# d-justen/duckdb-polr

Measured on AMD Instinct MI355X. Metric: probe-tuples/s, higher is better.
Workload: dtype u64

## Files before the change

duckdb-polr_amd/csrc/polr_flat_device.h:

```cpp
#pragma once

#include <hip/hip_runtime.h>
#include <stdint.h>

#include <type_traits>

#include "polr_device.h"

#define FLAT_STEP0 512
#define FLAT_UNIT_MAX 65536u

template <int K>
__device__ __host__ constexpr int flat_sweep_f() {
	return K <= 2 ? 8 : 4;
}
template <int K>
__device__ __host__ constexpr int flat_qcap() {
	return 64 * flat_sweep_f<K>() - 1 + 512;
}
template <int K>
__device__ __host__ constexpr int flat_qoff(int pos) {
	return (pos - 1) * (flat_qcap<K>() + 1);
}
template <int K>
__device__ __host__ constexpr int flat_per_wave_dwords() {
	return K <= 1 ? 0 : ((K - 1) * (flat_qcap<K>() + 1) * 2 + 3) / 4;
}

struct FlatStage {
	const POLR_GLOBAL uint32_t *keys;
	const POLR_GLOBAL uint8_t *valid;
	const POLR_GLOBAL uint32_t *table;
	uint32_t kind_lds;
	uint32_t a, b;
	uint32_t out_slot;
};

__device__ __forceinline__ FlatStage flat_load_stage(const StageDesc *d_generic, uint32_t join_index) {
	const POLR_GLOBAL StageDesc *d = as_global(d_generic);
	FlatStage s;
	s.out_slot = 1u + join_index;
	s.keys = as_global(uniptr((const uint32_t *)d->key_data[0]));
	s.valid = as_global(uniptr(d->key_valid[0]));
	s.table = as_global(uniptr((const uint32_t *)d->table));
	const uint32_t kind = uni(d->kind);
	s.kind_lds = kind | (uni(d->lds_off1) << 8);
	s.a = kind == KIND_PERFECT ? uni((uint32_t)d->min_value) : uni((uint32_t)d->mask);
	s.b = uni((uint32_t)d->range);
	return s;
}

template <int K>
struct FlatCtx {
	uint32_t k, lane;
	FlatStage st[K];
	const POLR_GLOBAL uint32_t *sel;
	const POLR_LDS uint32_t *lds_tables;
	POLR_LDS uint16_t *q;
	uint32_t qsize[K], cnt[K];
	uint64_t unit_begin, in_pos, in_end;
	DevOut out;
	OutState os;
	POLR_LDS unsigned long long *fused_lds;
	uint4 pf0, pf1;
	uint64_t pf_pos;
};

template <int F>
__device__ __forceinline__ void flat_perfect_issue(const FlatStage &s, const POLR_LDS uint32_t *lds_tables, const uint32_t (&key)[F],
                                                   const bool (&act)[F], uint32_t (&idx)[F], uint32_t (&w)[F]) {
	const uint32_t lds_off1 = s.kind_lds >> 8;
	bool in[F];
#pragma unroll
	for (int i = 0; i < F; i++) {
		idx[i] = key[i] - s.a;
		in[i] = act[i] && idx[i] <= s.b;
		w[i] = 0;
	}
	if (lds_off1) {
		const POLR_LDS uint32_t *bits = lds_tables + (lds_off1 - 1u);
#pragma unroll
		for (int i = 0; i < F; i++) {
			if (in[i]) {
				w[i] = bits[idx[i] >> 5];
			}
		}
	} else {
#pragma unroll
		for (int i = 0; i < F; i++) {
			if (in[i]) {
				w[i] = s.table[idx[i] >> 5];
			}
		}
	}
}

template <int F>
__device__ __forceinline__ void flat_hash_lookup(const FlatStage &s, const uint32_t (&key)[F], const bool (&act)[F],
                                                 bool (&hit)[F]) {
	const POLR_GLOBAL uint32_t *tab = s.table;
#pragma unroll
	for (int h0 = 0; h0 < F; h0 += 4) {
		uint32_t group[4], first[4];
		bool searching[4];
		bool any = false;
		const uint32_t gmask = s.a >> 2;
#pragma unroll
		for (int i = 0; i < 4; i++) {
			const uint64_t h = polr_murmurhash64((uint64_t)key[h0 + i]) & (uint64_t)s.a;
			group[i] = (uint32_t)(h >> 2);
			first[i] = (uint32_t)(h & 3u);
			searching[i] = act[h0 + i];
			hit[h0 + i] = false;
			any = any || searching[i];
		}
		while (__ballot(any) != 0ull) {
			uint4 a[4], b[4];
#pragma unroll
			for (int i = 0; i < 4; i++) {
				if (searching[i]) {
					a[i] = load_global_x4(tab + (uint64_t)group[i] * 8);
					b[i] = load_global_x4(tab + (uint64_t)group[i] * 8 + 4);
				}
			}
			any = false;
#pragma unroll
			for (int i = 0; i < 4; i++) {
				if (searching[i]) {
					const uint32_t kk[4] = {a[i].x, a[i].z, b[i].x, b[i].z};
					const uint32_t rr[4] = {a[i].y, a[i].w, b[i].y, b[i].w};
#pragma unroll
					for (int j = 0; j < 4; j++) {
						if (searching[i] && (uint32_t)j >= first[i]) {
							if (rr[j] == S8_EMPTY_ROW) {
								searching[i] = false;
							} else if (kk[j] == key[h0 + i]) {
								hit[h0 + i] = true;
								searching[i] = false;
							}
						}
					}
					first[i] = 0;
					group[i] = (group[i] + 1) & gmask;
				}
				any = any || searching[i];
			}
		}
	}
}

template <int F>
__device__ __forceinline__ void flat_lookup(const FlatStage &s, const POLR_LDS uint32_t *lds_tables, const uint32_t (&key)[F],
                                            const bool (&act)[F], bool (&hit)[F]) {
	if ((s.kind_lds & 0xFFu) == KIND_PERFECT) {
		uint32_t idx[F], w[F];
		flat_perfect_issue<F>(s, lds_tables, key, act, idx, w);
#pragma unroll
		for (int i = 0; i < F; i++) {
			hit[i] = (w[i] >> (idx[i] & 31u)) & 1u;
		}
	} else {
		flat_hash_lookup<F>(s, key, act, hit);
	}
}

#ifndef POLR_FLAT_EMIT
#define POLR_FLAT_EMIT 0
#endif
template <int K>
__device__ __forceinline__ void flat_fused_accumulate(FlatCtx<K> &c, uint32_t row) {
	const FusedSink *f = c.out.fused;
	auto slot_row = [&](uint32_t slot) {
		uint32_t r = row;
#pragma unroll
		for (int p = 0; p < K; p++) {
			if (p < (int)c.k && c.st[p].out_slot == slot) {
				r = c.st[p].keys[row] - c.st[p].a;
			}
		}
		return r;
	};
	uint64_t g = 0;
	bool ok = true;
	for (uint32_t q = 0; q < f->groups.n; q++) {
		const DevGroupKey gk = f->groups.k[q];
		const uint32_t r = slot_row(gk.slot);
		if (gk.src.valid && !as_global(gk.src.valid)[r]) {
			ok = false;
			break;
		}
		const unsigned long long off = (unsigned long long)(load_col_cell(gk.src, r) - gk.min_value);
		if (off >= gk.n_values) {
			ok = false;
			break;
		}
		g = g * gk.n_values + off;
	}
	if (!ok) {
		__hip_atomic_fetch_add(f->dropped, 1ull, __ATOMIC_RELAXED, __HIP_MEMORY_SCOPE_AGENT);
		return;
	}
	const uint32_t n_aggs = f->aggs.n;
	const size_t at = g * (1u + 2u * n_aggs);
	unsigned long long *gcell = f->cells + (size_t)(blockIdx.x % f->n_tables) * f->words_per_table + at;
	POLR_LDS unsigned long long *lcell = c.fused_lds + at;
	const bool in_lds = c.fused_lds != nullptr;
	auto add = [&](uint32_t w, unsigned long long v) {
		if (in_lds) {
			__hip_atomic_fetch_add(&lcell[w], v, __ATOMIC_RELAXED, __HIP_MEMORY_SCOPE_WORKGROUP);
		} else {
			__hip_atomic_fetch_add(&gcell[w], v, __ATOMIC_RELAXED, __HIP_MEMORY_SCOPE_AGENT);
		}
	};
	add(0, 1ull);
	for (uint32_t a = 0; a < n_aggs; a++) {
		const DevAgg ag = f->aggs.a[a];
		if (ag.fn == POLR_DEV_AGG_COUNT_STAR) {
			continue;
		}
		const uint32_t r = slot_row(ag.slot);
		if (ag.src.valid) {
			if (!as_global(ag.src.valid)[r]) {
				continue;
			}
			add(2u + 2u * a, 1ull);
		}
		if (ag.fn == POLR_DEV_AGG_SUM) {
			add(1u + 2u * a, (unsigned long long)load_col_cell(ag.src, r));
		}
	}
}

template <int K>
__device__ __forceinline__ void flat_out_write(FlatCtx<K> &c, uint32_t pos, bool valid) {
	const uint64_t m = __ballot(valid);
	const uint32_t n = (uint32_t)__popcll(m);
	if (n == 0) {
		return;
	}
	POLR_GLOBAL uint32_t *ids = as_global(c.out.ids);
	uint32_t row = 0, id[K];
	if (valid) {
		const uint64_t tp = c.unit_begin + pos;
		row = c.sel ? c.sel[tp] : (uint32_t)tp;
	}
	if (c.out.fused) {
		if (valid) {
			flat_fused_accumulate<K>(c, row);
		}
		return;
	}
	if (valid) {
#pragma unroll
		for (int p = 0; p < K; p++) {
			id[p] = p < (int)c.k ? c.st[p].keys[row] - c.st[p].a : 0u;
		}
	}
	out_claim(c.out, c.os, c.lane, m, valid, [&](uint64_t place) {
		ids[place] = row;
#pragma unroll
		for (int p = 0; p < K; p++) {
			if (p < (int)c.k) {
				ids[(uint64_t)c.st[p].out_slot * c.out.slot_stride + place] = id[p];
			}
		}
	});
}

template <int K, int POS, int F>
__device__ __forceinline__ void flat_emit(FlatCtx<K> &c, const uint32_t (&pos)[F], const bool (&hit)[F]) {
	const bool last = POS + 1 >= K || POS + 1 == (int)c.k;
	uint32_t total = 0;
#if POLR_FLAT_EMIT
	if (last && c.os.emit) {
#pragma unroll 1
		for (int i = 0; i < F; i++) {
			uint32_t p_i = pos[0];
			bool h_i = hit[0];
#pragma unroll
			for (int j = 1; j < F; j++) {
				p_i = j == i ? pos[j] : p_i;
				h_i = j == i ? hit[j] : h_i;
			}
			flat_out_write<K>(c, p_i, h_i);
		}
	}
#endif
	if constexpr (POS + 1 < K) {
		POLR_LDS uint16_t *qq = c.q + flat_qoff<K>(POS + 1);
		uint32_t qs = c.qsize[POS + 1];
#pragma unroll
		for (int i = 0; i < F; i++) {
			const uint64_t m = __ballot(hit[i]);
			const uint32_t n = (uint32_t)__popcll(m);
			if (!last && hit[i]) {
				qq[qs + lane_rank(m)] = (uint16_t)pos[i];
			}
			qs += n;
			total += n;
		}
		if (!last) {
			c.qsize[POS + 1] = qs;
		}
	} else {
#pragma unroll
		for (int i = 0; i < F; i++) {
			total += (uint32_t)__popcll(__ballot(hit[i]));
		}
	}
	c.cnt[POS] += total;
}

template <int K>
__device__ __forceinline__ void flat_stage0(FlatCtx<K> &c) {
	constexpr int F = 4;
	const FlatStage &s = c.st[0];
	const uint64_t left = c.in_end - c.in_pos;
	const uint32_t n = left < FLAT_STEP0 ? (uint32_t)left : (uint32_t)FLAT_STEP0;
	const uint32_t upos = (uint32_t)(c.in_pos - c.unit_begin);
	const bool streamable = c.sel == nullptr && s.valid == nullptr && (c.in_pos & 3ull) == 0 && (((uint64_t)s.keys) & 15ull) == 0;
	if (n == FLAT_STEP0 && streamable) {
		const uint32_t base = (uint32_t)c.in_pos + 4u * c.lane;
		uint4 kk[2];
		if (c.pf_pos == c.in_pos) {
			kk[0] = c.pf0;
			kk[1] = c.pf1;
		} else {
			kk[0] = load_global_x4(s.keys + base);
			kk[1] = load_global_x4(s.keys + base + 256u);
		}
		if (c.in_end - c.in_pos >= 2ull * FLAT_STEP0) {
			c.pf0 = load_global_x4(s.keys + base + FLAT_STEP0);
			c.pf1 = load_global_x4(s.keys + base + FLAT_STEP0 + 256u);
			c.pf_pos = c.in_pos + FLAT_STEP0;
		} else {
			c.pf_pos = ~0ull;
		}
		c.in_pos += n;
#pragma unroll
		for (int h = 0; h < 2; h++) {
			const uint32_t key[F] = {kk[h].x, kk[h].y, kk[h].z, kk[h].w};
			uint32_t pos[F];
			bool act[F], hit[F];
#pragma unroll
			for (int i = 0; i < F; i++) {
				pos[i] = upos + 4u * c.lane + h * 256u + i;
				act[i] = true;
			}
			flat_lookup<F>(s, c.lds_tables, key, act, hit);
			flat_emit<K, 0, F>(c, pos, hit);
		}
		return;
	}
	c.pf_pos = ~0ull;
	const uint64_t pos0 = c.in_pos;
	c.in_pos += n;
#pragma unroll 1
	for (uint32_t h = 0; h * 256u < n; h++) {
		uint32_t pos[F], row[F], key[F];
		bool act[F], hit[F];
#pragma unroll
		for (int i = 0; i < F; i++) {
			const uint32_t off = h * 256u + c.lane + 64u * i;
			act[i] = off < n;
			pos[i] = upos + off;
			const uint64_t tp = pos0 + off;
			row[i] = act[i] ? (c.sel ? c.sel[tp] : (uint32_t)tp) : 0u;
		}
#pragma unroll
		for (int i = 0; i < F; i++) {
			key[i] = act[i] ? s.keys[row[i]] : 0u;
		}
		if (s.valid) {
#pragma unroll
			for (int i = 0; i < F; i++) {
				act[i] = act[i] && s.valid[row[i]] != 0;
			}
		}
		flat_lookup<F>(s, c.lds_tables, key, act, hit);
		flat_emit<K, 0, F>(c, pos, hit);
	}
}

template <int I, int N, class Fn>
__device__ __forceinline__ void flat_static_for(Fn &&fn) {
	if constexpr (I < N) {
		fn(std::integral_constant<int, I> {});
		flat_static_for<I + 1, N>(fn);
	}
}
template <int I, int N, class Fn>
__device__ __forceinline__ void flat_static_for_down(Fn &&fn) {
	if constexpr (I >= 1) {
		fn(std::integral_constant<int, I> {});
		flat_static_for_down<I - 1, N>(fn);
	}
}

template <int K>
__device__ __forceinline__ void flat_sweep(FlatCtx<K> &c) {
	constexpr int F = flat_sweep_f<K>();
	if constexpr (K > 1) {
		uint32_t pos[K - 1][F], key[K - 1][F], w[K - 1][F];
		flat_static_for<1, K>([&](auto P) {
			constexpr int p = decltype(P)::value;
			if (p < (int)c.k) {
				const FlatStage &s = c.st[p];
				const uint32_t qs = c.qsize[p];
				const uint32_t n = qs < (uint32_t)(64 * F) ? qs : (uint32_t)(64 * F);
				const uint32_t base = qs - n;
				const POLR_LDS uint16_t *qq = c.q + flat_qoff<K>(p);
				uint32_t row[F];
#pragma unroll
				for (int i = 0; i < F; i++) {
					const uint32_t off = c.lane + 64u * i;
					pos[p - 1][i] = off < n ? (uint32_t)qq[base + off] : 0xFFFFFFFFu;
				}
				c.qsize[p] = base;
				if (c.sel) {
#pragma unroll
					for (int i = 0; i < F; i++) {
						row[i] = pos[p - 1][i] != 0xFFFFFFFFu ? c.sel[c.unit_begin + pos[p - 1][i]] : 0u;
					}
				} else {
#pragma unroll
					for (int i = 0; i < F; i++) {
						row[i] = (uint32_t)c.unit_begin + pos[p - 1][i];
					}
				}
#pragma unroll
				for (int i = 0; i < F; i++) {
					key[p - 1][i] = pos[p - 1][i] != 0xFFFFFFFFu ? s.keys[row[i]] : 0u;
				}
				if (s.valid) {
#pragma unroll
					for (int i = 0; i < F; i++) {
						if (pos[p - 1][i] != 0xFFFFFFFFu && s.valid[row[i]] == 0) {
							pos[p - 1][i] = 0xFFFFFFFFu;
						}
					}
				}
			}
		});
		flat_static_for<1, K>([&](auto P) {
			constexpr int p = decltype(P)::value;
			if (p < (int)c.k && (c.st[p].kind_lds & 0xFFu) == KIND_PERFECT) {
				const FlatStage &s = c.st[p];
				const uint32_t lds_off1 = s.kind_lds >> 8;
				bool in[F];
#pragma unroll
				for (int i = 0; i < F; i++) {
					const uint32_t idx = key[p - 1][i] - s.a;
					in[i] = pos[p - 1][i] != 0xFFFFFFFFu && idx <= s.b;
					key[p - 1][i] = idx;
					w[p - 1][i] = 0;
				}
				if (lds_off1) {
					const POLR_LDS uint32_t *bits = c.lds_tables + (lds_off1 - 1u);
#pragma unroll
					for (int i = 0; i < F; i++) {
						if (in[i]) {
							w[p - 1][i] = bits[key[p - 1][i] >> 5];
						}
					}
				} else {
#pragma unroll
					for (int i = 0; i < F; i++) {
						if (in[i]) {
							w[p - 1][i] = s.table[key[p - 1][i] >> 5];
						}
					}
				}
#pragma unroll
				for (int i = 0; i < F; i++) {
					key[p - 1][i] &= 31u;
				}
			}
		});
		flat_static_for<1, K>([&](auto P) {
			constexpr int p = decltype(P)::value;
			if (p < (int)c.k && (c.st[p].kind_lds & 0xFFu) != KIND_PERFECT) {
				bool act[F], hit[F];
#pragma unroll
				for (int i = 0; i < F; i++) {
					act[i] = pos[p - 1][i] != 0xFFFFFFFFu;
				}
				flat_hash_lookup<F>(c.st[p], key[p - 1], act, hit);
#pragma unroll
				for (int i = 0; i < F; i++) {
					w[p - 1][i] = hit[i] ? 1u : 0u;
					key[p - 1][i] = 0;
				}
			}
		});
		flat_static_for_down<K - 1, K>([&](auto P) {
			constexpr int p = decltype(P)::value;
			if (p < (int)c.k) {
				bool hit[F];
#pragma unroll
				for (int i = 0; i < F; i++) {
					hit[i] = (w[p - 1][i] >> key[p - 1][i]) & 1u;
				}
				flat_emit<K, p, F>(c, pos[p - 1], hit);
			}
		});
	}
}

template <int K>
__device__ __forceinline__ void flat_run_source(FlatCtx<K> &c) {
	while (true) {
		bool deep_full = false;
#pragma unroll
		for (int p = 1; p < K; p++) {
			if (p < (int)c.k) {
				deep_full = deep_full || c.qsize[p] >= (uint32_t)(64 * flat_sweep_f<K>());
			}
		}
		if (deep_full) {
			flat_sweep<K>(c);
		} else if (c.in_pos < c.in_end) {
			flat_stage0<K>(c);
		} else {
			return;
		}
	}
}

template <int K>
__device__ __forceinline__ void flat_run_drain(FlatCtx<K> &c) {
	while (true) {
		bool deep_any = false;
#pragma unroll
		for (int p = 1; p < K; p++) {
			if (p < (int)c.k) {
				deep_any = deep_any || c.qsize[p] > 0;
			}
		}
		if (!deep_any) {
			return;
		}
		flat_sweep<K>(c);
	}
}

template <int K>
__device__ __forceinline__ void flat_prefetch_unit(FlatCtx<K> &c, uint64_t begin, uint32_t count) {
	const FlatStage &s = c.st[0];
	const bool streamable = c.sel == nullptr && s.valid == nullptr && (begin & 3ull) == 0 && (((uint64_t)s.keys) & 15ull) == 0;
	if (count >= (uint32_t)FLAT_STEP0 && streamable) {
		const uint32_t base = (uint32_t)begin + 4u * c.lane;
		c.pf0 = load_global_x4(s.keys + base);
		c.pf1 = load_global_x4(s.keys + base + 256u);
		c.pf_pos = begin;
	}
}
```

duckdb-polr_amd/csrc/polr_pool.hip:

```cpp
#include <hip/hip_runtime.h>
#include <stdint.h>
#include <stddef.h>

#include "polr_device.h"
#include "polr_mpx_device.h"

#ifndef POLR_K
#error "compile with -DPOLR_K=<compiled stage count>"
#endif

#ifndef POLR_FLAT_EMIT
#define POLR_FLAT_EMIT 0
#endif

#include "polr_pool_common.h"
#include "polr_flat_device.h"

static_assert(FLAT_STEP0 == POLR_POOL_GRAN_FLAT && FLAT_UNIT_MAX == POLR_POOL_UNIT_MAX, "the plan's unit sizes are the kernel's");

#define PASTE_TL2(a, b) a##b
#define PASTE_TL(a, b) PASTE_TL2(a, b)
#if !POLR_FLAT_EMIT
POOL_DIAG_ENTRY(PASTE_TL(polr_diag_router_k, POLR_K), PASTE_TL(polr_diag_timeline_set_k, POLR_K))
#endif

#if POLR_FLAT_EMIT
__device__ __forceinline__ void flat_fused_flush(const DevOut &out, POLR_LDS unsigned long long *fused_lds, uint32_t fused_words) {
	__syncthreads();
	const FusedSink *f = out.fused;
	unsigned long long *table = f->cells + (size_t)(blockIdx.x % f->n_tables) * f->words_per_table;
	for (uint32_t i = threadIdx.x; i < fused_words; i += blockDim.x) {
		const unsigned long long v = fused_lds[i];
		if (v) {
			__hip_atomic_fetch_add(&table[i], v, __ATOMIC_RELAXED, __HIP_MEMORY_SCOPE_AGENT);
		}
	}
}
#endif

template <int K, int EMIT>
__global__ __launch_bounds__(1024) void polr_pool_flat_kernel(const DevPipeline *__restrict__ pipe,
                                                              const ResidentExec *__restrict__ execs, PoolRun *run,
                                                              DevOut out, uint32_t lds_per_wave, uint32_t table_dwords,
                                                              uint32_t router_dwords, uint32_t fused_off, uint32_t fused_words) {
	extern __shared__ __attribute__((aligned(16))) uint32_t lds[];
	const uint32_t wave_in_block = threadIdx.x >> 6;
	const uint32_t k = uni(pipe->k);
	PoolRun rh;
	pool_load_run(run, rh);
	const PoolRole role = pool_role(rh);
	const bool router_block = blockIdx.x < rh.n_router_blocks;
#if POLR_FLAT_EMIT
	if (router_block) {
		fused_words = 0;
	}
	POLR_LDS unsigned long long *fused_lds = fused_words ? as_lds((unsigned long long *)(lds + fused_off)) : nullptr;
	for (uint32_t i = threadIdx.x; i < fused_words; i += blockDim.x) {
		fused_lds[i] = 0ull;
	}
#endif
	{
		const uint32_t n_tab = router_block ? 0u : uni(pipe->n_lds_tables);
		for (uint32_t t = 0; t < n_tab; t++) {
			const uint32_t *src = uniptr(pipe->lds_table_src[t]);
			const uint32_t off = uni(pipe->lds_table_off[t]);
			const uint32_t len = uni(pipe->lds_table_len[t]);
			for (uint32_t i = threadIdx.x; i < len; i += blockDim.x) {
				lds[off + i] = src[i];
			}
		}
		__syncthreads();
	}
	if (role.router) {
		const uint32_t area = router_block ? router_dwords : POOL_ROUTER_MIN_DWORDS;
		uint32_t *base = lds + (router_block ? 0u : table_dwords + (blockDim.x >> 6) * lds_per_wave) + role.router_index * area;
		pool_router_wave(execs, run, rh, role.exec, k, FLAT_STEP0, base, area);
#if POLR_FLAT_EMIT
		if (fused_words) {
			flat_fused_flush(out, fused_lds, fused_words);
		}
#endif
		return;
	}
	const uint32_t pool_wave = role.pool_wave;
	const uint32_t ring = pool_wave & (rh.n_rings - 1u);
	FlatCtx<K> c;
	c.k = k;
	c.lane = threadIdx.x & 63;
	c.sel = as_global(uniptr(pipe->sel));
	c.lds_tables = as_lds((const uint32_t *)lds);
	c.q = as_lds((uint16_t *)(lds + table_dwords + (size_t)wave_in_block * lds_per_wave));
#pragma unroll
	for (int p = 0; p < K; p++) {
		c.qsize[p] = c.cnt[p] = 0;
		c.st[p].keys = nullptr;
		c.st[p].valid = nullptr;
		c.st[p].table = nullptr;
		c.st[p].kind_lds = c.st[p].a = c.st[p].b = c.st[p].out_slot = 0;
	}
	c.out = out;
	c.os = out_state_init();
#if POLR_FLAT_EMIT
	c.fused_lds = fused_lds;
#else
	c.fused_lds = nullptr;
#endif
	c.unit_begin = c.in_pos = c.in_end = 0;
	c.pf_pos = ~0ull;
	c.pf0 = make_uint4(0, 0, 0, 0);
	c.pf1 = make_uint4(0, 0, 0, 0);
	const StageDesc *stages = uniptr(pipe->stages);
	uint32_t cur_path = 0xFFFFFFFFu;
	PoolUnit u, nxt;
	PoolPoller pp;
	polr_pool_poller_init(pp, run, rh.sync, ring, rh.lo_cap, rh.hi_cap, pool_wave / rh.n_rings, rh.hi_lottery, rh.idle_sleep,
	                      rh.timeout_ticks);
	TL_BEGIN(pool_wave)
	bool have = polr_pool_next_unit(pp, u, c.lane);
	while (have) {
		TL_GOT
		if (u.path != cur_path) {
			c.pf_pos = ~0ull;
#pragma unroll
			for (int p = 0; p < K; p++) {
				if (p < (int)k) {
					c.st[p] = flat_load_stage(stages + (uint64_t)u.path * POLR_KMAX + p, uni(pipe->paths[u.path].order[p]));
				}
			}
			cur_path = u.path;
		}
#if POLR_FLAT_EMIT
		c.os.emit = u.emit != 0 && out.ids != nullptr && !c.os.overflow;
#endif
		c.unit_begin = u.begin;
		c.in_pos = u.begin;
		c.in_end = (uint64_t)u.begin + u.count;
		if (c.pf_pos != c.in_pos) {
			c.pf_pos = ~0ull;
		}
		flat_run_source<K>(c);
		const uint32_t peek = polr_pool_poll(pp, nxt, c.lane);
		if (peek == POLR_POLL_WORK && nxt.path == cur_path) {
			flat_prefetch_unit<K>(c, nxt.begin, nxt.count);
		}
		flat_run_drain<K>(c);
		TL_RUN
		pool_arrive<K>(execs, u, ring, c.k, c.cnt, c.lane);
		TL_DONE(u)
		if (peek == POLR_POLL_NONE) {
			have = polr_pool_next_unit(pp, nxt, c.lane);
		} else {
			have = peek == POLR_POLL_WORK;
		}
		u = nxt;
	}
#if POLR_FLAT_EMIT
	out_close(out, c.os, c.lane);
	if (fused_words) {
		flat_fused_flush(out, fused_lds, fused_words);
	}
#endif
}

#define PASTE2(a, b) a##b
#define PASTE(a, b) PASTE2(a, b)

static size_t pool_flat_wave_dwords() {
	return (size_t)flat_per_wave_dwords<POLR_K>();
}

static size_t pool_flat_lds_dwords(uint32_t waves_per_block, uint32_t table_dwords) {
	const size_t probe = table_dwords + pool_flat_wave_dwords() * waves_per_block;
	const size_t room = probe < POOL_LDS_DWORDS_MAX ? (POOL_LDS_DWORDS_MAX - probe) / POOL_ROUTER_MIN_DWORDS : 0;
	const size_t mixed = probe + (size_t)POOL_ROUTER_MIN_DWORDS * (room < POOL_ROUTER_RESERVE ? room : POOL_ROUTER_RESERVE);
	const size_t router = (size_t)POOL_ROUTER_MIN_DWORDS * waves_per_block;
	return mixed > router ? mixed : router;
}

static size_t pool_flat_launch_lds(uint32_t waves_per_block, uint32_t table_dwords, uint32_t fused_words, uint32_t *fused_off) {
	const size_t dwords = pool_flat_lds_dwords(waves_per_block, table_dwords);
	const uint32_t off = (uint32_t)((dwords + 1) & ~(size_t)1);
	if (fused_off) {
		*fused_off = off;
	}
	return (fused_words ? (size_t)off + 2 * (size_t)fused_words : dwords) * sizeof(uint32_t);
}

static hipError_t pool_flat_prepare(size_t lds) {
	static size_t lds_set = 0;
	if (lds > lds_set) {
		hipError_t e = hipFuncSetAttribute((const void *)polr_pool_flat_kernel<POLR_K, POLR_FLAT_EMIT>,
		                                   hipFuncAttributeMaxDynamicSharedMemorySize, (int)lds);
		if (e != hipSuccess) {
			return e;
		}
		lds_set = lds;
	}
	return hipSuccess;
}

#if POLR_FLAT_EMIT
#define FLAT_EXPORT(name) PASTE(PASTE(name, e_k), POLR_K)
#else
#define FLAT_EXPORT(name) PASTE(PASTE(name, k), POLR_K)
#endif

#if !POLR_FLAT_EMIT
extern "C++" size_t PASTE(polr_pool_flat_lds_bytes_k, POLR_K)(uint32_t waves_per_block, uint32_t table_dwords) {
	return pool_flat_lds_dwords(waves_per_block, table_dwords) * sizeof(uint32_t);
}

extern "C++" size_t PASTE(polr_pool_flat_wave_bytes_k, POLR_K)() {
	return pool_flat_wave_dwords() * sizeof(uint32_t);
}

extern "C++" uint32_t PASTE(polr_pool_flat_router_areas_k, POLR_K)(uint32_t waves_per_block, uint32_t table_dwords) {
	const size_t probe = table_dwords + pool_flat_wave_dwords() * waves_per_block;
	const size_t areas = (pool_flat_lds_dwords(waves_per_block, table_dwords) - probe) / POOL_ROUTER_MIN_DWORDS;
	return (uint32_t)(areas < POOL_ROUTER_RESERVE ? areas : POOL_ROUTER_RESERVE);
}
#endif

extern "C++" int FLAT_EXPORT(polr_pool_flat_occupancy_)(uint32_t waves_per_block, uint32_t table_dwords, uint32_t fused_words) {
	const size_t lds = pool_flat_launch_lds(waves_per_block, table_dwords, fused_words, nullptr);
	int blocks = 0;
	if (pool_flat_prepare(lds) != hipSuccess ||
	    hipOccupancyMaxActiveBlocksPerMultiprocessor(&blocks, (const void *)polr_pool_flat_kernel<POLR_K, POLR_FLAT_EMIT>,
	                                                 (int)(64 * waves_per_block), lds) != hipSuccess) {
		return 0;
	}
	return blocks;
}

extern "C++" hipError_t FLAT_EXPORT(polr_launch_pool_flat_kernel_)(uint32_t n_blocks, uint32_t waves_per_block,
                                                                      uint32_t table_dwords, hipStream_t stream,
                                                                      const DevPipeline *pipe, const ResidentExec *execs,
                                                                      PoolRun *run, DevOut out, uint32_t fused_words) {
	const size_t dwords = pool_flat_lds_dwords(waves_per_block, table_dwords);
	uint32_t fused_off = 0;
	const size_t lds = pool_flat_launch_lds(waves_per_block, table_dwords, fused_words, &fused_off);
	hipError_t e = pool_flat_prepare(lds);
	if (e != hipSuccess) {
		return e;
	}
	uint32_t per_wave = (uint32_t)pool_flat_wave_dwords();
	uint32_t router_dwords = (uint32_t)(dwords / waves_per_block);
	dim3 grid(n_blocks), block(64 * waves_per_block);
	uint32_t fused_off_arg = fused_words ? fused_off : 0u;
	void *args[] = {(void *)&pipe,         (void *)&execs,         (void *)&run,           (void *)&out,        (void *)&per_wave,
	                (void *)&table_dwords, (void *)&router_dwords, (void *)&fused_off_arg, (void *)&fused_words};
	return hipLaunchKernel((const void *)polr_pool_flat_kernel<POLR_K, POLR_FLAT_EMIT>, grid, block, args, lds, stream);
}
```

Measured before the change: 453.1 billion.

## Make probe loads branch-free and batch key gathers across stages before table lookups

Replaces per-lane predicated loads in the perfect-hash lookup and the stage-0/sweep gathers with unconditional loads using clamped indices, so all memory requests can be issued back-to-back without exec-mask branches. The sweep is restructured to pop all stage queues, gather selection rows, keys and validity bytes for every stage in one batch, then issue table lookups. A per-path 'plain' fast path skips the selection and validity handling when neither is present. Packing the bit index into the high bits of pos saves registers. Unconditional loads touch clamped addresses and add some memory traffic, and explicit waitcnt and asm barriers constrain compiler scheduling.

```diff
diff --git a/duckdb-polr_amd/csrc/polr_flat_device.h b/duckdb-polr_amd/csrc/polr_flat_device.h
--- a/duckdb-polr_amd/csrc/polr_flat_device.h
+++ b/duckdb-polr_amd/csrc/polr_flat_device.h
@@ -55,6 +55,7 @@
 	uint32_t k, lane;
 	FlatStage st[K];
 	const POLR_GLOBAL uint32_t *sel;
+	bool plain;
 	const POLR_LDS uint32_t *lds_tables;
 	POLR_LDS uint16_t *q;
 	uint32_t qsize[K], cnt[K];
@@ -66,31 +67,27 @@
 	uint64_t pf_pos;
 };
 
+#define FLAT_NO_IDX 0xFFFFFFFFu
 template <int F>
 __device__ __forceinline__ void flat_perfect_issue(const FlatStage &s, const POLR_LDS uint32_t *lds_tables, const uint32_t (&key)[F],
                                                    const bool (&act)[F], uint32_t (&idx)[F], uint32_t (&w)[F]) {
 	const uint32_t lds_off1 = s.kind_lds >> 8;
-	bool in[F];
+	uint32_t at[F];
 #pragma unroll
 	for (int i = 0; i < F; i++) {
-		idx[i] = key[i] - s.a;
-		in[i] = act[i] && idx[i] <= s.b;
-		w[i] = 0;
+		idx[i] = act[i] ? key[i] - s.a : FLAT_NO_IDX;
+		at[i] = (idx[i] < s.b ? idx[i] : s.b) >> 5;
 	}
 	if (lds_off1) {
 		const POLR_LDS uint32_t *bits = lds_tables + (lds_off1 - 1u);
 #pragma unroll
 		for (int i = 0; i < F; i++) {
-			if (in[i]) {
-				w[i] = bits[idx[i] >> 5];
-			}
+			w[i] = bits[at[i]];
 		}
 	} else {
 #pragma unroll
 		for (int i = 0; i < F; i++) {
-			if (in[i]) {
-				w[i] = s.table[idx[i] >> 5];
-			}
+			w[i] = s.table[at[i]];
 		}
 	}
 }
@@ -157,7 +154,7 @@
 		flat_perfect_issue<F>(s, lds_tables, key, act, idx, w);
 #pragma unroll
 		for (int i = 0; i < F; i++) {
-			hit[i] = (w[i] >> (idx[i] & 31u)) & 1u;
+			hit[i] = idx[i] <= s.b && ((w[i] >> (idx[i] & 31u)) & 1u) != 0;
 		}
 	} else {
 		flat_hash_lookup<F>(s, key, act, hit);
@@ -355,27 +352,43 @@
 	c.pf_pos = ~0ull;
 	const uint64_t pos0 = c.in_pos;
 	c.in_pos += n;
+	const bool has_valid = s.valid != nullptr;
+	const POLR_GLOBAL uint8_t *vbytes = has_valid ? s.valid : (const POLR_GLOBAL uint8_t *)s.keys;
+	const uint32_t vmask = has_valid ? 0xFFFFFFFFu : 0u;
+	const uint32_t no_valid = has_valid ? 0u : 1u;
 #pragma unroll 1
 	for (uint32_t h = 0; h * 256u < n; h++) {
-		uint32_t pos[F], row[F], key[F];
+		uint32_t pos[F], row[F], key[F], vb[F];
 		bool act[F], hit[F];
+		asm volatile("; polr-stage0-slow-begin" ::: "memory");
 #pragma unroll
 		for (int i = 0; i < F; i++) {
 			const uint32_t off = h * 256u + c.lane + 64u * i;
 			act[i] = off < n;
 			pos[i] = upos + off;
-			const uint64_t tp = pos0 + off;
-			row[i] = act[i] ? (c.sel ? c.sel[tp] : (uint32_t)tp) : 0u;
-		}
-#pragma unroll
-		for (int i = 0; i < F; i++) {
-			key[i] = act[i] ? s.keys[row[i]] : 0u;
-		}
-		if (s.valid) {
+			row[i] = act[i] ? off : 0u;
+		}
+		if (c.sel) {
 #pragma unroll
 			for (int i = 0; i < F; i++) {
-				act[i] = act[i] && s.valid[row[i]] != 0;
-			}
+				row[i] = c.sel[pos0 + row[i]];
+			}
+			__builtin_amdgcn_s_waitcnt(0x0F70);
+		} else {
+#pragma unroll
+			for (int i = 0; i < F; i++) {
+				row[i] += (uint32_t)pos0;
+			}
+		}
+#pragma unroll
+		for (int i = 0; i < F; i++) {
+			key[i] = s.keys[row[i]];
+			vb[i] = vbytes[row[i] & vmask];
+		}
+		asm volatile("; polr-stage0-slow-end" ::: "memory");
+#pragma unroll
+		for (int i = 0; i < F; i++) {
+			act[i] = act[i] && (vb[i] | no_valid) != 0;
 		}
 		flat_lookup<F>(s, c.lds_tables, key, act, hit);
 		flat_emit<K, 0, F>(c, pos, hit);
@@ -397,99 +410,145 @@
 	}
 }
 
+#define FLAT_INACTIVE 0xFFFFFFFFu
+
+template <int K, int P, int F>
+__device__ __forceinline__ void flat_pop(FlatCtx<K> &c, uint32_t (&pos)[F]) {
+	const uint32_t qs = c.qsize[P];
+	const uint32_t n = qs < (uint32_t)(64 * F) ? qs : (uint32_t)(64 * F);
+	const uint32_t base = qs - n;
+	const POLR_LDS uint16_t *qq = c.q + flat_qoff<K>(P);
+#pragma unroll
+	for (int i = 0; i < F; i++) {
+		const uint32_t off = c.lane + 64u * i;
+		const uint32_t e = qq[base + (off < n ? off : 0u)];
+		pos[i] = off < n ? e : FLAT_INACTIVE;
+	}
+	c.qsize[P] = base;
+}
+
+template <int F>
+__device__ __forceinline__ void flat_await(const uint32_t (&v)[F]) {
+	static_assert(F == 4 || F == 8, "sweep widths");
+	if constexpr (F == 4) {
+		asm volatile("; polr-sweep-await" ::"v"(v[0]), "v"(v[1]), "v"(v[2]), "v"(v[3]));
+	} else {
+		asm volatile("; polr-sweep-await" ::"v"(v[0]), "v"(v[1]), "v"(v[2]), "v"(v[3]), "v"(v[4]), "v"(v[5]), "v"(v[6]), "v"(v[7]));
+	}
+}
+
 template <int K>
 __device__ __forceinline__ void flat_sweep(FlatCtx<K> &c) {
 	constexpr int F = flat_sweep_f<K>();
 	if constexpr (K > 1) {
-		uint32_t pos[K - 1][F], key[K - 1][F], w[K - 1][F];
-		flat_static_for<1, K>([&](auto P) {
-			constexpr int p = decltype(P)::value;
-			if (p < (int)c.k) {
-				const FlatStage &s = c.st[p];
-				const uint32_t qs = c.qsize[p];
-				const uint32_t n = qs < (uint32_t)(64 * F) ? qs : (uint32_t)(64 * F);
-				const uint32_t base = qs - n;
-				const POLR_LDS uint16_t *qq = c.q + flat_qoff<K>(p);
-				uint32_t row[F];
-#pragma unroll
-				for (int i = 0; i < F; i++) {
-					const uint32_t off = c.lane + 64u * i;
-					pos[p - 1][i] = off < n ? (uint32_t)qq[base + off] : 0xFFFFFFFFu;
-				}
-				c.qsize[p] = base;
-				if (c.sel) {
+		uint32_t pos[K - 1][F], key[K - 1][F];
+		if (c.plain) {
+			asm volatile("; polr-sweep-keys-begin" ::: "memory");
+			flat_static_for<1, K>([&](auto P) {
+				constexpr int p = decltype(P)::value;
+				const POLR_GLOBAL uint32_t *keys = (p < (int)c.k ? c.st[p].keys : c.st[0].keys) + (uint32_t)c.unit_begin;
+				flat_pop<K, p, F>(c, pos[p - 1]);
+#pragma unroll
+				for (int i = 0; i < F; i++) {
+					key[p - 1][i] = keys[pos[p - 1][i] != FLAT_INACTIVE ? pos[p - 1][i] : 0u];
+				}
+			});
+			asm volatile("; polr-sweep-keys-end" ::: "memory");
+		} else {
+			uint32_t vb[K - 1][F];
+			asm volatile("; polr-sweep-sel-keys-begin" ::: "memory");
+			flat_static_for<1, K>([&](auto P) {
+				constexpr int p = decltype(P)::value;
+				flat_pop<K, p, F>(c, pos[p - 1]);
+#pragma unroll
+				for (int i = 0; i < F; i++) {
+					key[p - 1][i] = pos[p - 1][i] != FLAT_INACTIVE ? pos[p - 1][i] : 0u;
+				}
+			});
+			if (c.sel) {
+				flat_static_for<1, K>([&](auto P) {
+					constexpr int p = decltype(P)::value;
 #pragma unroll
 					for (int i = 0; i < F; i++) {
-						row[i] = pos[p - 1][i] != 0xFFFFFFFFu ? c.sel[c.unit_begin + pos[p - 1][i]] : 0u;
+						key[p - 1][i] = c.sel[c.unit_begin + key[p - 1][i]];
 					}
-				} else {
+				});
+				__builtin_amdgcn_s_waitcnt(0x0F70);
+			} else {
+				flat_static_for<1, K>([&](auto P) {
+					constexpr int p = decltype(P)::value;
 #pragma unroll
 					for (int i = 0; i < F; i++) {
-						row[i] = (uint32_t)c.unit_begin + pos[p - 1][i];
+						key[p - 1][i] += (uint32_t)c.unit_begin;
 					}
-				}
-#pragma unroll
-				for (int i = 0; i < F; i++) {
-					key[p - 1][i] = pos[p - 1][i] != 0xFFFFFFFFu ? s.keys[row[i]] : 0u;
-				}
-				if (s.valid) {
-#pragma unroll
-					for (int i = 0; i < F; i++) {
-						if (pos[p - 1][i] != 0xFFFFFFFFu && s.valid[row[i]] == 0) {
-							pos[p - 1][i] = 0xFFFFFFFFu;
-						}
-					}
-				}
-			}
-		});
+				});
+			}
+			flat_static_for<1, K>([&](auto P) {
+				constexpr int p = decltype(P)::value;
+				const bool live = p < (int)c.k;
+				const POLR_GLOBAL uint32_t *keys = live ? c.st[p].keys : c.st[0].keys;
+				const bool has_valid = live && c.st[p].valid != nullptr;
+				const POLR_GLOBAL uint8_t *vbytes = has_valid ? c.st[p].valid : (const POLR_GLOBAL uint8_t *)keys;
+				const uint32_t vmask = has_valid ? 0xFFFFFFFFu : 0u;
+#pragma unroll
+				for (int i = 0; i < F; i++) {
+					const uint32_t row = key[p - 1][i];
+					vb[p - 1][i] = vbytes[row & vmask];
+					key[p - 1][i] = keys[row];
+				}
+			});
+			asm volatile("; polr-sweep-sel-keys-end" ::: "memory");
+			flat_static_for<1, K>([&](auto P) {
+				constexpr int p = decltype(P)::value;
+				const uint32_t no_valid = p < (int)c.k && c.st[p].valid != nullptr ? 0u : 1u;
+#pragma unroll
+				for (int i = 0; i < F; i++) {
+					pos[p - 1][i] = (vb[p - 1][i] | no_valid) != 0 ? pos[p - 1][i] : FLAT_INACTIVE;
+				}
+			});
+		}
+		flat_static_for<1, K>([&](auto P) { flat_await<F>(key[decltype(P)::value - 1]); });
+		asm volatile("; polr-sweep-tables-begin" ::: "memory");
 		flat_static_for<1, K>([&](auto P) {
 			constexpr int p = decltype(P)::value;
 			if (p < (int)c.k && (c.st[p].kind_lds & 0xFFu) == KIND_PERFECT) {
 				const FlatStage &s = c.st[p];
 				const uint32_t lds_off1 = s.kind_lds >> 8;
-				bool in[F];
+				uint32_t at[F];
 #pragma unroll
 				for (int i = 0; i < F; i++) {
 					const uint32_t idx = key[p - 1][i] - s.a;
-					in[i] = pos[p - 1][i] != 0xFFFFFFFFu && idx <= s.b;
-					key[p - 1][i] = idx;
-					w[p - 1][i] = 0;
+					const bool in = pos[p - 1][i] != FLAT_INACTIVE && idx <= s.b;
+					pos[p - 1][i] = in ? pos[p - 1][i] | ((idx & 31u) << 16) : FLAT_INACTIVE;
+					at[i] = (idx < s.b ? idx : s.b) >> 5;
 				}
 				if (lds_off1) {
 					const POLR_LDS uint32_t *bits = c.lds_tables + (lds_off1 - 1u);
 #pragma unroll
 					for (int i = 0; i < F; i++) {
-						if (in[i]) {
-							w[p - 1][i] = bits[key[p - 1][i] >> 5];
-						}
+						key[p - 1][i] = bits[at[i]];
 					}
 				} else {
 #pragma unroll
 					for (int i = 0; i < F; i++) {
-						if (in[i]) {
-							w[p - 1][i] = s.table[key[p - 1][i] >> 5];
-						}
+						key[p - 1][i] = s.table[at[i]];
 					}
 				}
-#pragma unroll
-				for (int i = 0; i < F; i++) {
-					key[p - 1][i] &= 31u;
-				}
 			}
 		});
+		asm volatile("; polr-sweep-tables-end" ::: "memory");
 		flat_static_for<1, K>([&](auto P) {
 			constexpr int p = decltype(P)::value;
 			if (p < (int)c.k && (c.st[p].kind_lds & 0xFFu) != KIND_PERFECT) {
 				bool act[F], hit[F];
 #pragma unroll
 				for (int i = 0; i < F; i++) {
-					act[i] = pos[p - 1][i] != 0xFFFFFFFFu;
+					act[i] = pos[p - 1][i] != FLAT_INACTIVE;
 				}
 				flat_hash_lookup<F>(c.st[p], key[p - 1], act, hit);
 #pragma unroll
 				for (int i = 0; i < F; i++) {
-					w[p - 1][i] = hit[i] ? 1u : 0u;
-					key[p - 1][i] = 0;
+					key[p - 1][i] = hit[i] ? 1u : 0u;
 				}
 			}
 		});
@@ -499,12 +558,23 @@
 				bool hit[F];
 #pragma unroll
 				for (int i = 0; i < F; i++) {
-					hit[i] = (w[p - 1][i] >> key[p - 1][i]) & 1u;
+					hit[i] = pos[p - 1][i] != FLAT_INACTIVE && ((key[p - 1][i] >> ((pos[p - 1][i] >> 16) & 31u)) & 1u) != 0;
+					pos[p - 1][i] &= 0xFFFFu;
 				}
 				flat_emit<K, p, F>(c, pos[p - 1], hit);
 			}
 		});
 	}
+}
+
+template <int K>
+__device__ __forceinline__ void flat_set_plain(FlatCtx<K> &c) {
+	bool plain = c.sel == nullptr;
+#pragma unroll
+	for (int p = 1; p < K; p++) {
+		plain = plain && !(p < (int)c.k && c.st[p].valid != nullptr);
+	}
+	c.plain = plain;
 }
 
 template <int K>
diff --git a/duckdb-polr_amd/csrc/polr_pool.hip b/duckdb-polr_amd/csrc/polr_pool.hip
--- a/duckdb-polr_amd/csrc/polr_pool.hip
+++ b/duckdb-polr_amd/csrc/polr_pool.hip
@@ -88,6 +88,7 @@
 	c.k = k;
 	c.lane = threadIdx.x & 63;
 	c.sel = as_global(uniptr(pipe->sel));
+	c.plain = false;
 	c.lds_tables = as_lds((const uint32_t *)lds);
 	c.q = as_lds((uint16_t *)(lds + table_dwords + (size_t)wave_in_block * lds_per_wave));
 #pragma unroll
@@ -127,6 +128,7 @@
 					c.st[p] = flat_load_stage(stages + (uint64_t)u.path * POLR_KMAX + p, uni(pipe->paths[u.path].order[p]));
 				}
 			}
+			flat_set_plain<K>(c);
 			cur_path = u.path;
 		}
 #if POLR_FLAT_EMIT
```

Measured after the change: 476.4 billion (median of 6 runs). 5.1% higher.
